# ActiveVisionLab/CrossScore

Measured on AMD Instinct MI355X. Metric: query-images/sec at 518x518, 5 ref views, bs=8; score-map MAE vs ref, higher is better.
Workload: dtype fp16

## Files before the change

### crossscore_amd/build.py

```python
from __future__ import annotations

import os
import subprocess
import sys

HERE = os.path.dirname(os.path.abspath(__file__))
CSRC = os.path.join(HERE, "csrc")
LIB = os.path.join(HERE, "libcrossscore_hip.so")
SOURCES = ["api.hip", "forward.hip", "ops.hip", "fit_host.hip", "gemm.hip", "gemm256.hip", "attention.hip", "refuse.hip", "elementwise.hip", "preprocess.hip", "panel.hip", "panel4.hip", "patch.hip", "rowln.hip", "png.hip", "pngdec.hip", "jpegdec.hip", "jpegprog.hip", "gtmap.hip", "gtsum.hip", "select.hip", "scorepool.hip", "sheet.hip", "headfit.hip", "tailfit.hip", "attnbwd.hip", "crossfit.hip", "layerfit.hip"]


EXTRA_FLAGS = {"panel.hip": ["-fno-slp-vectorize"], "panel4.hip": ["-fno-slp-vectorize"], "attention.hip": ["-fno-slp-vectorize"]}


def _hipcc() -> str:
    for c in (os.environ.get("HIPCC"), "/opt/rocm/bin/hipcc", "hipcc"):
        if c and (os.path.isabs(c) and os.path.exists(c) or not os.path.isabs(c)):
            return c
    return "hipcc"


def needs_build() -> bool:
    if not os.path.exists(LIB):
        return True
    t = os.path.getmtime(LIB)
    deps = [os.path.join(CSRC, f) for f in os.listdir(CSRC)] + [os.path.join(os.path.dirname(HERE), "include", "crossscore_hip.h")]
    return any(os.path.getmtime(d) > t for d in deps)


def compile_library(lib: str, extra=None, csrc: str = CSRC, objdir=None, verbose: bool = True) -> str:
    objdir = objdir or os.path.join(HERE, "build")
    os.makedirs(objdir, exist_ok=True)
    objs = []
    procs = []
    for s in SOURCES:
        o = os.path.join(objdir, s.replace(".hip", ".o"))
        objs.append(o)
        cmd = ([_hipcc(), "--offload-arch=gfx950", "-O3", "-std=c++17", "-fPIC", "-Wno-unused-value"] + EXTRA_FLAGS.get(s, []) + (extra or {}).get(s, []) +
               ["-c", os.path.join(csrc, s), "-o", o])
        procs.append((cmd, subprocess.Popen(cmd, stdout=subprocess.PIPE, stderr=subprocess.STDOUT, text=True)))
    for cmd, p in procs:
        out, _ = p.communicate()
        if p.returncode != 0:
            raise RuntimeError("hipcc failed: " + " ".join(cmd) + "\n" + out)
        if verbose and out.strip():
            print(out, file=sys.stderr)
    cmd = [_hipcc(), "--offload-arch=gfx950", "-shared", "-fPIC", "-o", lib] + objs
    r = subprocess.run(cmd, stdout=subprocess.PIPE, stderr=subprocess.STDOUT, text=True)
    if r.returncode != 0:
        raise RuntimeError("link failed: " + r.stdout)
    return lib


def build(force: bool = False, verbose: bool = True) -> str:
    if not force and not needs_build():
        return LIB
    return compile_library(LIB, verbose=verbose)


if __name__ == "__main__":
    print(build(force="--force" in sys.argv))
```

### crossscore_amd/csrc/rowln.hip

```cpp
#include "cs_common.h"
#include <atomic>

namespace {

__device__ __forceinline__ float rl_add_other_half(float x) {
  const auto r = __builtin_amdgcn_permlane32_swap(__float_as_uint(x), __float_as_uint(x), false, false);
  return __uint_as_float(r[0]) + __uint_as_float(r[1]);
}

template <int C, bool BF, int G2>
__global__ __launch_bounds__(C / 96 * 64) void cs_rowln_kernel(CsRowLnParams p) {
  constexpr int NW = C / 96, NT = NW * 64;
  constexpr bool NEXT = G2 > 0;
  constexpr int BK = 64, NSL = C / BK;
  constexpr int APITCH = C * 2 + 16;
  constexpr int WPITCH = BK * 2 + 16;
  constexpr int WBUF = C * WPITCH;
  constexpr int ACH = C / 8, WCH = BK / 8;
  constexpr int AIT = 64 * ACH / NT, WIT = C * WCH / NT;
  static_assert(64 * ACH % NT == 0 && C * WCH % NT == 0, "staging maps");
  extern __shared__ __attribute__((aligned(16))) char smem[];
  char* As = smem;
  char* Ws = smem + 64 * APITCH;
  float* red = reinterpret_cast<float*>(Ws + 2 * WBUF);
  const int tid = threadIdx.x;
  const int lane = tid & 63;
  const int wv = __builtin_amdgcn_readfirstlane(tid >> 6);
  const int j = lane & 31, h = lane >> 5;
  const int row0 = blockIdx.x * 64;
  const int col0 = wv * 96;
  uint4 wreg[WIT];
#define RL_LOAD_W(REG, WP, LDW, SL)                                                                                \
  _Pragma("unroll") for (int it = 0; it < WIT; ++it) {                                                         \
    const int c_ = tid + it * NT, r_ = c_ / WCH, ch_ = c_ - r_ * WCH;                                          \
    REG[it] = *reinterpret_cast<const uint4*>((WP) + (size_t)r_ * (LDW) + (SL) * BK + ch_ * 8);                \
  }
#define RL_WRITE_W(REG, BUF)                                                                                   \
  _Pragma("unroll") for (int it = 0; it < WIT; ++it) {                                                         \
    const int c_ = tid + it * NT, r_ = c_ / WCH, ch_ = c_ - r_ * WCH;                                          \
    *reinterpret_cast<uint4*>(Ws + (BUF) * WBUF + r_ * WPITCH + ch_ * 16) = REG[it];                           \
  }
  RL_LOAD_W(wreg, p.W, p.ldw, 0)
  {
    uint4 areg[AIT];
#pragma unroll
    for (int it = 0; it < AIT; ++it) {
      const int c = tid + it * NT, r = c / ACH, ch = c - r * ACH;
      areg[it] = *reinterpret_cast<const uint4*>(p.A + (size_t)min(row0 + r, p.M - 1) * p.lda + ch * 8);
    }
#pragma unroll
    for (int it = 0; it < AIT; ++it) {
      const int c = tid + it * NT, r = c / ACH, ch = c - r * ACH;
      *reinterpret_cast<uint4*>(As + r * APITCH + ch * 16) = areg[it];
    }
  }
#define RL_KSLICE(SLICE)                                                                                       \
  _Pragma("unroll") for (int ks = 0; ks < BK / 16; ++ks) {                                                     \
    h16x8_t a[2], w[3];                                                                                        \
    _Pragma("unroll") for (int rb = 0; rb < 2; ++rb)                                                           \
      a[rb] = *reinterpret_cast<const h16x8_t*>(a_rd + rb * 32 * APITCH + ((SLICE) * (BK / 16) + ks) * 32);    \
    _Pragma("unroll") for (int ct = 0; ct < 3; ++ct) w[ct] = *reinterpret_cast<const h16x8_t*>(w_rd + ct * 32 * WPITCH + ks * 32); \
    _Pragma("unroll") for (int rb = 0; rb < 2; ++rb)                                                           \
      _Pragma("unroll") for (int ct = 0; ct < 3; ++ct) acc[rb][ct] = mfma_32x32x16<BF>(w[ct], a[rb], acc[rb][ct]); \
  }
  RL_WRITE_W(wreg, 0)
  __syncthreads();
  f32x16_t acc[2][3];
#pragma unroll
  for (int rb = 0; rb < 2; ++rb)
#pragma unroll
    for (int ct = 0; ct < 3; ++ct)
#pragma unroll
      for (int e = 0; e < 16; ++e) acc[rb][ct][e] = 0.f;
  const char* a_rd = As + j * APITCH + h * 16;
  for (int sl = 0; sl < NSL; ++sl) {
    if (sl + 1 < NSL) { RL_LOAD_W(wreg, p.W, p.ldw, sl + 1) }
    const char* w_rd = Ws + (sl & 1) * WBUF + (col0 + j) * WPITCH + h * 16;
    RL_KSLICE(sl)
    if (sl + 1 < NSL) { RL_WRITE_W(wreg, (sl + 1) & 1) }
    __syncthreads();
  }
  f32x4_t gam[3][4], bet[3][4];
#pragma unroll
  for (int ct = 0; ct < 3; ++ct)
#pragma unroll
    for (int g = 0; g < 4; ++g) {
      const int c = col0 + 32 * ct + 8 * g + 4 * h;
      const f32x4_t b4 = *reinterpret_cast<const f32x4_t*>(p.bias + c);
      gam[ct][g] = *reinterpret_cast<const f32x4_t*>(p.gamma + c);
      bet[ct][g] = *reinterpret_cast<const f32x4_t*>(p.beta + c);
#pragma unroll
      for (int rb = 0; rb < 2; ++rb)
#pragma unroll
        for (int i = 0; i < 4; ++i) acc[rb][ct][4 * g + i] += b4[i];
    }
  if (p.resid) {
#pragma unroll
    for (int rb = 0; rb < 2; ++rb) {
      const float* rr = p.resid + (size_t)min(row0 + 32 * rb + j, p.M - 1) * p.ldr + col0 + 4 * h;
#pragma unroll
      for (int ct = 0; ct < 3; ++ct)
#pragma unroll
        for (int g = 0; g < 4; ++g) {
          const f32x4_t r4 = *reinterpret_cast<const f32x4_t*>(rr + 32 * ct + 8 * g);
#pragma unroll
          for (int i = 0; i < 4; ++i) acc[rb][ct][4 * g + i] += r4[i];
        }
    }
  }
  float mean[2], rstd[2];
#pragma unroll
  for (int rb = 0; rb < 2; ++rb) {
    float s = 0.f;
#pragma unroll
    for (int ct = 0; ct < 3; ++ct)
#pragma unroll
      for (int e = 0; e < 16; e += 4) s += (acc[rb][ct][e] + acc[rb][ct][e + 1]) + (acc[rb][ct][e + 2] + acc[rb][ct][e + 3]);
    s = rl_add_other_half(s);
    if (h == 0) red[(0 * NW + wv) * 64 + 32 * rb + j] = s;
  }
  __syncthreads();
#pragma unroll
  for (int rb = 0; rb < 2; ++rb) {
    float s = 0.f;
#pragma unroll
    for (int w2 = 0; w2 < NW; ++w2) s += red[(0 * NW + w2) * 64 + 32 * rb + j];
    mean[rb] = s * (1.0f / C);
    float q = 0.f;
#pragma unroll
    for (int ct = 0; ct < 3; ++ct)
#pragma unroll
      for (int e = 0; e < 16; ++e) {
        const float d = acc[rb][ct][e] - mean[rb];
        q = fmaf(d, d, q);
      }
    q = rl_add_other_half(q);
    if (h == 0) red[(1 * NW + wv) * 64 + 32 * rb + j] = q;
  }
  __syncthreads();
#pragma unroll
  for (int rb = 0; rb < 2; ++rb) {
    float q = 0.f;
#pragma unroll
    for (int w2 = 0; w2 < NW; ++w2) q += red[(1 * NW + w2) * 64 + 32 * rb + j];
    rstd[rb] = 1.0f / sqrtf(q * (1.0f / C) + p.eps);
  }
#pragma unroll
  for (int rb = 0; rb < 2; ++rb) {
    const int row = row0 + 32 * rb + j;
    if (row < p.M) {
      float* o32 = p.out_f32 ? p.out_f32 + (size_t)row * C + col0 + 4 * h : nullptr;
      h16_t* o16 = p.out_f16 ? p.out_f16 + (size_t)row * C + col0 + 4 * h : nullptr;
#pragma unroll
      for (int ct = 0; ct < 3; ++ct)
#pragma unroll
        for (int g = 0; g < 4; ++g) {
          f32x4_t y;
#pragma unroll
          for (int i = 0; i < 4; ++i) y[i] = (acc[rb][ct][4 * g + i] - mean[rb]) * rstd[rb] * gam[ct][g][i] + bet[ct][g][i];
          if (o32) *reinterpret_cast<f32x4_t*>(o32 + 32 * ct + 8 * g) = y;
          if (o16) {
            uint2 o;
            o.x = pack_o16x2<BF>(y[0], y[1]);
            o.y = pack_o16x2<BF>(y[2], y[3]);
            *reinterpret_cast<uint2*>(o16 + 32 * ct + 8 * g) = o;
          }
        }
    }
  }
  if constexpr (NEXT) {
#pragma unroll
    for (int rb = 0; rb < 2; ++rb) {
      char* arow = As + (32 * rb + j) * APITCH + (col0 + 4 * h) * 2;
#pragma unroll
      for (int ct = 0; ct < 3; ++ct)
#pragma unroll
        for (int g = 0; g < 4; ++g) {
          float y[4];
#pragma unroll
          for (int i = 0; i < 4; ++i) y[i] = (acc[rb][ct][4 * g + i] - mean[rb]) * rstd[rb] * gam[ct][g][i] + bet[ct][g][i];
          uint2 o;
          o.x = pack_o16x2<BF>(y[0], y[1]);
          o.y = pack_o16x2<BF>(y[2], y[3]);
          *reinterpret_cast<uint2*>(arow + (32 * ct + 8 * g) * 2) = o;
        }
    }
    RL_LOAD_W(wreg, p.W2, p.ldw2, 0)
    RL_WRITE_W(wreg, 0)
    __syncthreads();
    constexpr int nsl2 = G2 * NSL;
#pragma unroll
    for (int s2 = 0; s2 < nsl2; ++s2) {
      const int grp = s2 / NSL, sl = s2 - grp * NSL;
      if (sl == 0) {
#pragma unroll
        for (int rb = 0; rb < 2; ++rb)
#pragma unroll
          for (int ct = 0; ct < 3; ++ct)
#pragma unroll
            for (int e = 0; e < 16; ++e) acc[rb][ct][e] = 0.f;
      }
      if (s2 + 1 < nsl2) {
        const int g2 = (s2 + 1) / NSL, sn = (s2 + 1) - g2 * NSL;
        RL_LOAD_W(wreg, p.W2 + (size_t)g2 * C * p.ldw2, p.ldw2, sn)
      }
      const char* w_rd = Ws + (s2 & 1) * WBUF + (col0 + j) * WPITCH + h * 16;
      RL_KSLICE(sl)
      if (s2 + 1 < nsl2) { RL_WRITE_W(wreg, (s2 + 1) & 1) }
      __syncthreads();
      if (sl == NSL - 1) {
#pragma unroll
        for (int rb = 0; rb < 2; ++rb) {
          const int row = row0 + 32 * rb + j;
          if (row < p.M) {
            h16_t* o2 = p.out2 + (size_t)row * p.ld2 + grp * C + col0 + 4 * h;
            const float* b2 = p.bias2 + grp * C + col0 + 4 * h;
#pragma unroll
            for (int ct = 0; ct < 3; ++ct)
#pragma unroll
              for (int g = 0; g < 4; ++g) {
                const f32x4_t b4 = *reinterpret_cast<const f32x4_t*>(b2 + 32 * ct + 8 * g);
                float v[4];
#pragma unroll
                for (int i = 0; i < 4; ++i) {
                  v[i] = acc[rb][ct][4 * g + i] + b4[i];
                  if (p.act2 == 1) v[i] = fmaxf(v[i], 0.f);
                  if (p.act2 == 2) v[i] = v[i] >= 0.f ? v[i] : 0.01f * v[i];
                }
                uint2 o;
                o.x = pack_o16x2<BF>(v[0], v[1]);
                o.y = pack_o16x2<BF>(v[2], v[3]);
                *reinterpret_cast<uint2*>(o2 + 32 * ct + 8 * g) = o;
              }
          }
        }
      }
    }
  }
#undef RL_KSLICE
#undef RL_LOAD_W
#undef RL_WRITE_W
}

}

extern "C" int cs_rowln_supported(int C) { return C == 384; }

extern "C" const char* cs_rowln_check(const CsRowLnParams* p, int C) {
  if (!cs_rowln_supported(C)) return "linear + LayerNorm: built for C = 384";
  if (!p->A || !p->W || !p->bias || !p->gamma || !p->beta || (!p->out_f32 && !p->out_f16 && !p->n2)) return "linear + LayerNorm: null operand";
  if (p->n2) {
    if ((p->n2 != C && p->n2 != 3 * C) || p->act2 < 0 || p->act2 > 2) return "linear + LayerNorm: the second stage takes C or 3 C output columns and act2 in 0..2";
    if (!p->W2 || !p->bias2 || !p->out2) return "linear + LayerNorm: null operand (second stage)";
    if (p->ldw2 % 8 || p->ldw2 < C || p->ld2 % 4 || p->ld2 < p->n2) return "linear + LayerNorm: row strides must keep 16-byte rows (second stage)";
    if (((uintptr_t)p->W2 | (uintptr_t)p->bias2) & 15 || ((uintptr_t)p->out2 & 7)) return "linear + LayerNorm: operands must be 16-byte aligned (second stage)";
  }
  if (p->M <= 0) return "linear + LayerNorm: empty shape";
  if (p->lda % 8 || p->ldw % 8 || p->lda < C || p->ldw < C || (p->resid && (p->ldr % 4 || p->ldr < C))) return "linear + LayerNorm: row strides must keep 16-byte rows";
  if (((uintptr_t)p->A | (uintptr_t)p->W | (uintptr_t)p->bias | (uintptr_t)p->gamma | (uintptr_t)p->beta | (uintptr_t)p->resid | (uintptr_t)p->out_f32 |
       (uintptr_t)p->out_f16) & 15)
    return "linear + LayerNorm: operands must be 16-byte aligned";
  return nullptr;
}

extern "C" hipError_t cs_rowln_launch(const CsRowLnParams* p, int C, int bf16, hipStream_t st) {
  if (C != 384) return hipErrorInvalidValue;
  constexpr int CC = 384, NW = CC / 96;
  constexpr int lds = 64 * (CC * 2 + 16) + 2 * CC * (64 * 2 + 16) + 2 * NW * 64 * 4;
  static std::atomic<bool> attr_done[16];
  int dev = 0;
  if (hipGetDevice(&dev) != hipSuccess || dev < 0 || dev >= 16) return hipErrorInvalidDevice;
  if (!attr_done[dev]) {
    const void* fns[6] = {reinterpret_cast<const void*>(cs_rowln_kernel<384, true, 0>), reinterpret_cast<const void*>(cs_rowln_kernel<384, false, 0>),
                          reinterpret_cast<const void*>(cs_rowln_kernel<384, true, 1>), reinterpret_cast<const void*>(cs_rowln_kernel<384, false, 1>),
                          reinterpret_cast<const void*>(cs_rowln_kernel<384, true, 3>), reinterpret_cast<const void*>(cs_rowln_kernel<384, false, 3>)};
    for (const void* f : fns)
      if (hipError_t e = hipFuncSetAttribute(f, hipFuncAttributeMaxDynamicSharedMemorySize, lds); e != hipSuccess) return e;
    attr_done[dev] = true;
  }
  const dim3 grid((p->M + 63) / 64), block(NW * 64);
#define RL_GO(G) do { if (bf16) hipLaunchKernelGGL((cs_rowln_kernel<384, true, G>), grid, block, lds, st, *p);  \
                      else hipLaunchKernelGGL((cs_rowln_kernel<384, false, G>), grid, block, lds, st, *p); } while (0)
  if (p->n2 == 0) RL_GO(0);
  else if (p->n2 == CC) RL_GO(1);
  else if (p->n2 == 3 * CC) RL_GO(3);
  else return hipErrorInvalidValue;
#undef RL_GO
  return hipGetLastError();
}
```

Before: 1397.

## Rewrite fused linear+LayerNorm kernel with per-wave DMA weight ring and 16x16 MFMA tiles

Restructures the row-LayerNorm GEMM kernel from 4 waves over 64-row tiles with register-staged, double-buffered weight slices into 8 waves over 48-row tiles. Each wave streams its own weight columns through a 4-deep per-wave LDS ring using direct global-to-LDS loads, synchronised with explicit vmcnt/lgkm waits instead of block-wide syncthreads. Both stages, including the chained second GEMM, run as one fully unrolled compile-time pipeline, and MFMA switches from 32x32x16 to 16x16x32. The intent is to hide weight-load latency and cut barrier overhead and register pressure, at the cost of heavy inline asm, hand-counted wait values that are fragile, and more blocks with smaller row tiles.

```diff
diff --git a/crossscore_amd/build.py b/crossscore_amd/build.py
--- a/crossscore_amd/build.py
+++ b/crossscore_amd/build.py
@@ -10,7 +10,8 @@
 SOURCES = ["api.hip", "forward.hip", "ops.hip", "fit_host.hip", "gemm.hip", "gemm256.hip", "attention.hip", "refuse.hip", "elementwise.hip", "preprocess.hip", "panel.hip", "panel4.hip", "patch.hip", "rowln.hip", "png.hip", "pngdec.hip", "jpegdec.hip", "jpegprog.hip", "gtmap.hip", "gtsum.hip", "select.hip", "scorepool.hip", "sheet.hip", "headfit.hip", "tailfit.hip", "attnbwd.hip", "crossfit.hip", "layerfit.hip"]
 
 
-EXTRA_FLAGS = {"panel.hip": ["-fno-slp-vectorize"], "panel4.hip": ["-fno-slp-vectorize"], "attention.hip": ["-fno-slp-vectorize"]}
+EXTRA_FLAGS = {"panel.hip": ["-fno-slp-vectorize"], "panel4.hip": ["-fno-slp-vectorize"], "attention.hip": ["-fno-slp-vectorize"],
+               "rowln.hip": ["-fno-slp-vectorize"]}
 
 
 def _hipcc() -> str:
diff --git a/crossscore_amd/csrc/rowln.hip b/crossscore_amd/csrc/rowln.hip
--- a/crossscore_amd/csrc/rowln.hip
+++ b/crossscore_amd/csrc/rowln.hip
@@ -1,245 +1,252 @@
-#include "cs_common.h"
+#include "panel_shared.h"
 #include <atomic>
 
 namespace {
 
-__device__ __forceinline__ float rl_add_other_half(float x) {
-  const auto r = __builtin_amdgcn_permlane32_swap(__float_as_uint(x), __float_as_uint(x), false, false);
-  return __uint_as_float(r[0]) + __uint_as_float(r[1]);
+constexpr int RL_R = 48;
+constexpr int RL_NW = 8;
+constexpr int RL_BK = 32;
+constexpr int RL_NS = 4;
+constexpr int RL_D = RL_NS - 1;
+constexpr int RL_SLOT = 3 * PANEL_FRAG;
+
+template <int C> struct RlCfg {
+  static_assert(C == RL_NW * 48 && C % RL_BK == 0, "eight waves of 48 columns");
+  static constexpr int NSL = C / RL_BK;
+  static constexpr int A_BYTES = 3 * NSL * PANEL_FRAG;
+  static constexpr int RING_OFF = A_BYTES;
+  static constexpr int RED_OFF = RING_OFF + RL_NW * RL_NS * RL_SLOT;
+  static constexpr int LDS = RED_OFF + 2 * RL_NW * RL_R * 4;
+};
+
+typedef unsigned rl_u32x2_t __attribute__((ext_vector_type(2)));
+
+__device__ __forceinline__ float rl_add_groups(float x) {
+  const auto r = __builtin_amdgcn_permlane16_swap(__float_as_uint(x), __float_as_uint(x), false, false);
+  return add_other_half(__uint_as_float(r[0]) + __uint_as_float(r[1]));
+}
+__device__ __forceinline__ void rl_gload16(f32x4_t& r, const float* src) {
+  asm volatile("global_load_dwordx4 %0, %1, off" : "=v"(r) : "v"(src) : "memory");
+}
+__device__ __forceinline__ void rl_touch(f32x4_t& r) { asm volatile("" : "+v"(r)); }
+__device__ __forceinline__ void rl_lds_write4(unsigned addr, float v) { asm volatile("ds_write_b32 %0, %1" ::"v"(addr), "v"(v) : "memory"); }
+__device__ __forceinline__ void rl_lds_write8(unsigned addr, rl_u32x2_t v) { asm volatile("ds_write_b64 %0, %1" ::"v"(addr), "v"(v) : "memory"); }
+template <int OFF>
+__device__ __forceinline__ void rl_lds_read4(unsigned addr, float& v) {
+  asm volatile("ds_read_b32 %0, %1 offset:%2" : "=&v"(v) : "v"(addr), "n"(OFF) : "memory");
+}
+__device__ __forceinline__ float rl_sum_waves(unsigned addr) {
+  float x[RL_NW];
+  sfor<RL_NW>([&](auto w) { rl_lds_read4<decltype(w)::value * RL_R * 4>(addr, x[decltype(w)::value]); });
+  CS_LGKM(0);
+  return ((x[0] + x[1]) + (x[2] + x[3])) + ((x[4] + x[5]) + (x[6] + x[7]));
 }
 
 template <int C, bool BF, int G2>
-__global__ __launch_bounds__(C / 96 * 64) void cs_rowln_kernel(CsRowLnParams p) {
-  constexpr int NW = C / 96, NT = NW * 64;
+__global__ __launch_bounds__(RL_NW * 64) void cs_rowln_kernel(CsRowLnParams p) {
+  using Cfg = RlCfg<C>;
   constexpr bool NEXT = G2 > 0;
-  constexpr int BK = 64, NSL = C / BK;
-  constexpr int APITCH = C * 2 + 16;
-  constexpr int WPITCH = BK * 2 + 16;
-  constexpr int WBUF = C * WPITCH;
-  constexpr int ACH = C / 8, WCH = BK / 8;
-  constexpr int AIT = 64 * ACH / NT, WIT = C * WCH / NT;
-  static_assert(64 * ACH % NT == 0 && C * WCH % NT == 0, "staging maps");
+  constexpr int NSL = Cfg::NSL, T = NSL * (1 + G2);
   extern __shared__ __attribute__((aligned(16))) char smem[];
-  char* As = smem;
-  char* Ws = smem + 64 * APITCH;
-  float* red = reinterpret_cast<float*>(Ws + 2 * WBUF);
+  const unsigned lds0 = (unsigned)(size_t)CS_LDS_PTR(smem);
   const int tid = threadIdx.x;
   const int lane = tid & 63;
   const int wv = __builtin_amdgcn_readfirstlane(tid >> 6);
-  const int j = lane & 31, h = lane >> 5;
-  const int row0 = blockIdx.x * 64;
-  const int col0 = wv * 96;
-  uint4 wreg[WIT];
-#define RL_LOAD_W(REG, WP, LDW, SL)                                                                                \
-  _Pragma("unroll") for (int it = 0; it < WIT; ++it) {                                                         \
-    const int c_ = tid + it * NT, r_ = c_ / WCH, ch_ = c_ - r_ * WCH;                                          \
-    REG[it] = *reinterpret_cast<const uint4*>((WP) + (size_t)r_ * (LDW) + (SL) * BK + ch_ * 8);                \
-  }
-#define RL_WRITE_W(REG, BUF)                                                                                   \
-  _Pragma("unroll") for (int it = 0; it < WIT; ++it) {                                                         \
-    const int c_ = tid + it * NT, r_ = c_ / WCH, ch_ = c_ - r_ * WCH;                                          \
-    *reinterpret_cast<uint4*>(Ws + (BUF) * WBUF + r_ * WPITCH + ch_ * 16) = REG[it];                           \
-  }
-  RL_LOAD_W(wreg, p.W, p.ldw, 0)
-  {
-    uint4 areg[AIT];
-#pragma unroll
-    for (int it = 0; it < AIT; ++it) {
-      const int c = tid + it * NT, r = c / ACH, ch = c - r * ACH;
-      areg[it] = *reinterpret_cast<const uint4*>(p.A + (size_t)min(row0 + r, p.M - 1) * p.lda + ch * 8);
-    }
-#pragma unroll
-    for (int it = 0; it < AIT; ++it) {
-      const int c = tid + it * NT, r = c / ACH, ch = c - r * ACH;
-      *reinterpret_cast<uint4*>(As + r * APITCH + ch * 16) = areg[it];
-    }
-  }
-#define RL_KSLICE(SLICE)                                                                                       \
-  _Pragma("unroll") for (int ks = 0; ks < BK / 16; ++ks) {                                                     \
-    h16x8_t a[2], w[3];                                                                                        \
-    _Pragma("unroll") for (int rb = 0; rb < 2; ++rb)                                                           \
-      a[rb] = *reinterpret_cast<const h16x8_t*>(a_rd + rb * 32 * APITCH + ((SLICE) * (BK / 16) + ks) * 32);    \
-    _Pragma("unroll") for (int ct = 0; ct < 3; ++ct) w[ct] = *reinterpret_cast<const h16x8_t*>(w_rd + ct * 32 * WPITCH + ks * 32); \
-    _Pragma("unroll") for (int rb = 0; rb < 2; ++rb)                                                           \
-      _Pragma("unroll") for (int ct = 0; ct < 3; ++ct) acc[rb][ct] = mfma_32x32x16<BF>(w[ct], a[rb], acc[rb][ct]); \
-  }
-  RL_WRITE_W(wreg, 0)
-  __syncthreads();
-  f32x16_t acc[2][3];
-#pragma unroll
-  for (int rb = 0; rb < 2; ++rb)
-#pragma unroll
-    for (int ct = 0; ct < 3; ++ct)
-#pragma unroll
-      for (int e = 0; e < 16; ++e) acc[rb][ct][e] = 0.f;
-  const char* a_rd = As + j * APITCH + h * 16;
-  for (int sl = 0; sl < NSL; ++sl) {
-    if (sl + 1 < NSL) { RL_LOAD_W(wreg, p.W, p.ldw, sl + 1) }
-    const char* w_rd = Ws + (sl & 1) * WBUF + (col0 + j) * WPITCH + h * 16;
-    RL_KSLICE(sl)
-    if (sl + 1 < NSL) { RL_WRITE_W(wreg, (sl + 1) & 1) }
-    __syncthreads();
-  }
-  f32x4_t gam[3][4], bet[3][4];
-#pragma unroll
-  for (int ct = 0; ct < 3; ++ct)
-#pragma unroll
-    for (int g = 0; g < 4; ++g) {
-      const int c = col0 + 32 * ct + 8 * g + 4 * h;
-      const f32x4_t b4 = *reinterpret_cast<const f32x4_t*>(p.bias + c);
-      gam[ct][g] = *reinterpret_cast<const f32x4_t*>(p.gamma + c);
-      bet[ct][g] = *reinterpret_cast<const f32x4_t*>(p.beta + c);
-#pragma unroll
-      for (int rb = 0; rb < 2; ++rb)
-#pragma unroll
-        for (int i = 0; i < 4; ++i) acc[rb][ct][4 * g + i] += b4[i];
-    }
-  if (p.resid) {
-#pragma unroll
-    for (int rb = 0; rb < 2; ++rb) {
-      const float* rr = p.resid + (size_t)min(row0 + 32 * rb + j, p.M - 1) * p.ldr + col0 + 4 * h;
-#pragma unroll
-      for (int ct = 0; ct < 3; ++ct)
-#pragma unroll
-        for (int g = 0; g < 4; ++g) {
-          const f32x4_t r4 = *reinterpret_cast<const f32x4_t*>(rr + 32 * ct + 8 * g);
-#pragma unroll
-          for (int i = 0; i < 4; ++i) acc[rb][ct][4 * g + i] += r4[i];
+  const int j = lane & 15, g = lane >> 4;
+  const int row0 = blockIdx.x * RL_R;
+  const int col0 = wv * 48;
+  const unsigned a_rd = lds0 + lane * 16;
+  const unsigned ring = lds0 + Cfg::RING_OFF + wv * (RL_NS * RL_SLOT);
+  const unsigned w_rd = ring + lane * 16;
+  const unsigned red = lds0 + Cfg::RED_OFF + (wv * RL_R + j) * 4;
+  const unsigned red_rd = lds0 + Cfg::RED_OFF + j * 4;
+
+  f32x4_t b4[3], gam[3], bet[3], r4[3][3], b2[NEXT ? G2 : 1][3];
+  int rowc[3];
+#pragma unroll
+  for (int rt = 0; rt < 3; ++rt) rowc[rt] = min(row0 + 16 * rt + j, p.M - 1);
+#pragma unroll
+  for (int ct = 0; ct < 3; ++ct) {
+    const int c = col0 + 16 * ct + 4 * g;
+    rl_gload16(b4[ct], p.bias + c);
+    rl_gload16(gam[ct], p.gamma + c);
+    rl_gload16(bet[ct], p.beta + c);
+  }
+#pragma unroll
+  for (int rt = 0; rt < 3; ++rt)
+#pragma unroll
+    for (int ct = 0; ct < 3; ++ct) {
+      const int c = col0 + 16 * ct + 4 * g;
+      rl_gload16(r4[rt][ct], p.resid ? p.resid + (size_t)rowc[rt] * p.ldr + c : p.bias + c);
+    }
+  if constexpr (NEXT) {
+#pragma unroll
+    for (int grp = 0; grp < G2; ++grp)
+#pragma unroll
+      for (int ct = 0; ct < 3; ++ct) rl_gload16(b2[grp][ct], p.bias2 + grp * C + col0 + 16 * ct + 4 * g);
+  }
+#pragma unroll
+  for (int rt = 0; rt < 3; ++rt) {
+    const char* src = reinterpret_cast<const char*>(p.A + (size_t)rowc[rt] * p.lda + 8 * g);
+    dma_piece<0>(src + wv * 64, lds0 + (rt * NSL + wv) * PANEL_FRAG);
+    if (wv < NSL - RL_NW) dma_piece<0>(src + (wv + RL_NW) * 64, lds0 + (rt * NSL + wv + RL_NW) * PANEL_FRAG);
+  }
+  const char* wsrc[3];
+  const char* w2src[3];
+#pragma unroll
+  for (int ct = 0; ct < 3; ++ct) {
+    wsrc[ct] = reinterpret_cast<const char*>(p.W + (size_t)(col0 + 16 * ct + j) * p.ldw + 8 * g);
+    w2src[ct] = NEXT ? reinterpret_cast<const char*>(p.W2 + (size_t)(col0 + 16 * ct + j) * p.ldw2 + 8 * g) : nullptr;
+  }
+  auto issue = [&](auto tc) {
+    constexpr int t = decltype(tc)::value;
+    if constexpr (t < T) {
+      constexpr int slot = t % RL_NS, grp = t < NSL ? 0 : (t - NSL) / NSL, s = t % NSL;
+      sfor<3>([&](auto ct_) {
+        constexpr int ct = decltype(ct_)::value;
+        const char* src = t < NSL ? wsrc[ct] + s * 64 : w2src[ct] + ((size_t)grp * C * p.ldw2 + s * RL_BK) * 2;
+        dma_piece<0>(src, ring + slot * RL_SLOT + ct * PANEL_FRAG);
+      });
+    }
+  };
+  h16x8_t wf[2][3], af[2][3];
+  auto read_frags = [&](auto tc) {
+    constexpr int t = decltype(tc)::value;
+    constexpr int slot = t % RL_NS, s = t % NSL, b = t & 1;
+    sfor<3>([&](auto i_) {
+      constexpr int i = decltype(i_)::value;
+      lds_read1<slot * RL_SLOT + i * PANEL_FRAG>(w_rd, wf[b][i]);
+      lds_read1<(i * NSL + s) * PANEL_FRAG>(a_rd, af[b][i]);
+    });
+  };
+  sfor<RL_D>([&](auto tc) { issue(tc); });
+  CS_VMCNT(3 * RL_D);
+  __builtin_amdgcn_s_barrier();
+#pragma unroll
+  for (int ct = 0; ct < 3; ++ct) {
+    rl_touch(b4[ct]); rl_touch(gam[ct]); rl_touch(bet[ct]);
+#pragma unroll
+    for (int rt = 0; rt < 3; ++rt) rl_touch(r4[rt][ct]);
+    if constexpr (NEXT) {
+#pragma unroll
+      for (int grp = 0; grp < G2; ++grp) rl_touch(b2[grp][ct]);
+    }
+  }
+  CS_VMCNT(3 * (RL_D - 1));
+  read_frags(IC<0>{});
+  CS_LGKM(0);
+
+  f32x4_t acc[3][3];
+  float mean[3], rstd[3];
+  sfor<T>([&](auto tc) {
+    constexpr int t = decltype(tc)::value;
+    constexpr int s = t % NSL;
+    constexpr bool ahead = t + 1 < T && t + 1 != NSL;
+    if constexpr (s == 0) {
+#pragma unroll
+      for (int rt = 0; rt < 3; ++rt)
+#pragma unroll
+        for (int ct = 0; ct < 3; ++ct) acc[rt][ct] = f32x4_t{0.f, 0.f, 0.f, 0.f};
+    }
+    issue(IC<t + RL_D>{});
+    if constexpr (ahead) {
+      constexpr int last = t + RL_D < T - 1 ? t + RL_D : T - 1;
+      CS_VMCNT(3 * (last - (t + 1)));
+      read_frags(IC<t + 1>{});
+      CS_SB();
+    }
+#pragma unroll
+    for (int rt = 0; rt < 3; ++rt)
+#pragma unroll
+      for (int ct = 0; ct < 3; ++ct) acc[rt][ct] = mfma_16x16x32<BF>(wf[t & 1][ct], af[t & 1][rt], acc[rt][ct]);
+    CS_SB();
+    CS_LGKM(0);
+
+    if constexpr (t == NSL - 1) {
+#pragma unroll
+      for (int rt = 0; rt < 3; ++rt)
+#pragma unroll
+        for (int ct = 0; ct < 3; ++ct) {
+          acc[rt][ct] += b4[ct];
+          if (p.resid) acc[rt][ct] += r4[rt][ct];
         }
-    }
-  }
-  float mean[2], rstd[2];
-#pragma unroll
-  for (int rb = 0; rb < 2; ++rb) {
-    float s = 0.f;
-#pragma unroll
-    for (int ct = 0; ct < 3; ++ct)
-#pragma unroll
-      for (int e = 0; e < 16; e += 4) s += (acc[rb][ct][e] + acc[rb][ct][e + 1]) + (acc[rb][ct][e + 2] + acc[rb][ct][e + 3]);
-    s = rl_add_other_half(s);
-    if (h == 0) red[(0 * NW + wv) * 64 + 32 * rb + j] = s;
-  }
-  __syncthreads();
-#pragma unroll
-  for (int rb = 0; rb < 2; ++rb) {
-    float s = 0.f;
-#pragma unroll
-    for (int w2 = 0; w2 < NW; ++w2) s += red[(0 * NW + w2) * 64 + 32 * rb + j];
-    mean[rb] = s * (1.0f / C);
-    float q = 0.f;
-#pragma unroll
-    for (int ct = 0; ct < 3; ++ct)
-#pragma unroll
-      for (int e = 0; e < 16; ++e) {
-        const float d = acc[rb][ct][e] - mean[rb];
-        q = fmaf(d, d, q);
-      }
-    q = rl_add_other_half(q);
-    if (h == 0) red[(1 * NW + wv) * 64 + 32 * rb + j] = q;
-  }
-  __syncthreads();
-#pragma unroll
-  for (int rb = 0; rb < 2; ++rb) {
-    float q = 0.f;
-#pragma unroll
-    for (int w2 = 0; w2 < NW; ++w2) q += red[(1 * NW + w2) * 64 + 32 * rb + j];
-    rstd[rb] = 1.0f / sqrtf(q * (1.0f / C) + p.eps);
-  }
-#pragma unroll
-  for (int rb = 0; rb < 2; ++rb) {
-    const int row = row0 + 32 * rb + j;
-    if (row < p.M) {
-      float* o32 = p.out_f32 ? p.out_f32 + (size_t)row * C + col0 + 4 * h : nullptr;
-      h16_t* o16 = p.out_f16 ? p.out_f16 + (size_t)row * C + col0 + 4 * h : nullptr;
-#pragma unroll
-      for (int ct = 0; ct < 3; ++ct)
-#pragma unroll
-        for (int g = 0; g < 4; ++g) {
+#pragma unroll
+      for (int rt = 0; rt < 3; ++rt) {
+        float part[3];
+#pragma unroll
+        for (int ct = 0; ct < 3; ++ct) part[ct] = (acc[rt][ct][0] + acc[rt][ct][1]) + (acc[rt][ct][2] + acc[rt][ct][3]);
+        const float sum = rl_add_groups((part[0] + part[1]) + part[2]);
+        if (g == 0) rl_lds_write4(red + 16 * rt * 4, sum);
+      }
+      CS_LGKM(0);
+      __builtin_amdgcn_s_barrier();
+#pragma unroll
+      for (int rt = 0; rt < 3; ++rt) {
+        mean[rt] = rl_sum_waves(red_rd + 16 * rt * 4) * (1.0f / C);
+        float q = 0.f;
+#pragma unroll
+        for (int ct = 0; ct < 3; ++ct)
+#pragma unroll
+          for (int i = 0; i < 4; ++i) {
+            const float d = acc[rt][ct][i] - mean[rt];
+            q = fmaf(d, d, q);
+          }
+        q = rl_add_groups(q);
+        if (g == 0) rl_lds_write4(red + (RL_NW * RL_R + 16 * rt) * 4, q);
+      }
+      CS_LGKM(0);
+      __builtin_amdgcn_s_barrier();
+#pragma unroll
+      for (int rt = 0; rt < 3; ++rt) rstd[rt] = 1.0f / sqrtf(rl_sum_waves(red_rd + (RL_NW * RL_R + 16 * rt) * 4) * (1.0f / C) + p.eps);
+#pragma unroll
+      for (int rt = 0; rt < 3; ++rt) {
+        const int row = row0 + 16 * rt + j;
+        float* o32 = p.out_f32 && row < p.M ? p.out_f32 + (size_t)row * C + col0 + 4 * g : nullptr;
+        h16_t* o16 = p.out_f16 && row < p.M ? p.out_f16 + (size_t)row * C + col0 + 4 * g : nullptr;
+#pragma unroll
+        for (int ct = 0; ct < 3; ++ct) {
           f32x4_t y;
 #pragma unroll
-          for (int i = 0; i < 4; ++i) y[i] = (acc[rb][ct][4 * g + i] - mean[rb]) * rstd[rb] * gam[ct][g][i] + bet[ct][g][i];
-          if (o32) *reinterpret_cast<f32x4_t*>(o32 + 32 * ct + 8 * g) = y;
-          if (o16) {
-            uint2 o;
-            o.x = pack_o16x2<BF>(y[0], y[1]);
-            o.y = pack_o16x2<BF>(y[2], y[3]);
-            *reinterpret_cast<uint2*>(o16 + 32 * ct + 8 * g) = o;
+          for (int i = 0; i < 4; ++i) y[i] = (acc[rt][ct][i] - mean[rt]) * rstd[rt] * gam[ct][i] + bet[ct][i];
+          const rl_u32x2_t o = {pack_o16x2<BF>(y[0], y[1]), pack_o16x2<BF>(y[2], y[3])};
+          if (o32) *reinterpret_cast<f32x4_t*>(o32 + 16 * ct) = y;
+          if (o16) *reinterpret_cast<rl_u32x2_t*>(o16 + 16 * ct) = o;
+          if constexpr (NEXT) {
+            const int f = col0 + 16 * ct + 4 * g;
+            rl_lds_write8(lds0 + (rt * NSL + (f >> 5)) * PANEL_FRAG + (j + 16 * ((f & 31) >> 3)) * 16 + (f & 7) * 2, o);
           }
         }
-    }
-  }
-  if constexpr (NEXT) {
-#pragma unroll
-    for (int rb = 0; rb < 2; ++rb) {
-      char* arow = As + (32 * rb + j) * APITCH + (col0 + 4 * h) * 2;
-#pragma unroll
-      for (int ct = 0; ct < 3; ++ct)
-#pragma unroll
-        for (int g = 0; g < 4; ++g) {
-          float y[4];
-#pragma unroll
-          for (int i = 0; i < 4; ++i) y[i] = (acc[rb][ct][4 * g + i] - mean[rb]) * rstd[rb] * gam[ct][g][i] + bet[ct][g][i];
-          uint2 o;
-          o.x = pack_o16x2<BF>(y[0], y[1]);
-          o.y = pack_o16x2<BF>(y[2], y[3]);
-          *reinterpret_cast<uint2*>(arow + (32 * ct + 8 * g) * 2) = o;
-        }
-    }
-    RL_LOAD_W(wreg, p.W2, p.ldw2, 0)
-    RL_WRITE_W(wreg, 0)
-    __syncthreads();
-    constexpr int nsl2 = G2 * NSL;
-#pragma unroll
-    for (int s2 = 0; s2 < nsl2; ++s2) {
-      const int grp = s2 / NSL, sl = s2 - grp * NSL;
-      if (sl == 0) {
-#pragma unroll
-        for (int rb = 0; rb < 2; ++rb)
-#pragma unroll
-          for (int ct = 0; ct < 3; ++ct)
-#pragma unroll
-            for (int e = 0; e < 16; ++e) acc[rb][ct][e] = 0.f;
-      }
-      if (s2 + 1 < nsl2) {
-        const int g2 = (s2 + 1) / NSL, sn = (s2 + 1) - g2 * NSL;
-        RL_LOAD_W(wreg, p.W2 + (size_t)g2 * C * p.ldw2, p.ldw2, sn)
-      }
-      const char* w_rd = Ws + (s2 & 1) * WBUF + (col0 + j) * WPITCH + h * 16;
-      RL_KSLICE(sl)
-      if (s2 + 1 < nsl2) { RL_WRITE_W(wreg, (s2 + 1) & 1) }
-      __syncthreads();
-      if (sl == NSL - 1) {
-#pragma unroll
-        for (int rb = 0; rb < 2; ++rb) {
-          const int row = row0 + 32 * rb + j;
-          if (row < p.M) {
-            h16_t* o2 = p.out2 + (size_t)row * p.ld2 + grp * C + col0 + 4 * h;
-            const float* b2 = p.bias2 + grp * C + col0 + 4 * h;
-#pragma unroll
-            for (int ct = 0; ct < 3; ++ct)
-#pragma unroll
-              for (int g = 0; g < 4; ++g) {
-                const f32x4_t b4 = *reinterpret_cast<const f32x4_t*>(b2 + 32 * ct + 8 * g);
-                float v[4];
-#pragma unroll
-                for (int i = 0; i < 4; ++i) {
-                  v[i] = acc[rb][ct][4 * g + i] + b4[i];
-                  if (p.act2 == 1) v[i] = fmaxf(v[i], 0.f);
-                  if (p.act2 == 2) v[i] = v[i] >= 0.f ? v[i] : 0.01f * v[i];
-                }
-                uint2 o;
-                o.x = pack_o16x2<BF>(v[0], v[1]);
-                o.y = pack_o16x2<BF>(v[2], v[3]);
-                *reinterpret_cast<uint2*>(o2 + 32 * ct + 8 * g) = o;
-              }
+      }
+      if constexpr (NEXT) {
+        CS_LGKM(0);
+        __builtin_amdgcn_s_barrier();
+        CS_VMCNT(3 * ((NSL - 1 + RL_D < T - 1 ? NSL - 1 + RL_D : T - 1) - NSL));
+        read_frags(IC<NSL>{});
+        CS_LGKM(0);
+      }
+    }
+    if constexpr (NEXT && t >= NSL && s == NSL - 1) {
+      constexpr int grp = (t - NSL) / NSL;
+#pragma unroll
+      for (int rt = 0; rt < 3; ++rt) {
+        const int row = row0 + 16 * rt + j;
+        if (row < p.M) {
+          h16_t* o2 = p.out2 + (size_t)row * p.ld2 + grp * C + col0 + 4 * g;
+#pragma unroll
+          for (int ct = 0; ct < 3; ++ct) {
+            float v[4];
+#pragma unroll
+            for (int i = 0; i < 4; ++i) {
+              v[i] = acc[rt][ct][i] + b2[grp][ct][i];
+              if (p.act2 == 1) v[i] = fmaxf(v[i], 0.f);
+              if (p.act2 == 2) v[i] = v[i] >= 0.f ? v[i] : 0.01f * v[i];
+            }
+            *reinterpret_cast<rl_u32x2_t*>(o2 + 16 * ct) = rl_u32x2_t{pack_o16x2<BF>(v[0], v[1]), pack_o16x2<BF>(v[2], v[3])};
           }
         }
       }
     }
-  }
-#undef RL_KSLICE
-#undef RL_LOAD_W
-#undef RL_WRITE_W
+  });
 }
 
 }
@@ -265,8 +272,7 @@
 
 extern "C" hipError_t cs_rowln_launch(const CsRowLnParams* p, int C, int bf16, hipStream_t st) {
   if (C != 384) return hipErrorInvalidValue;
-  constexpr int CC = 384, NW = CC / 96;
-  constexpr int lds = 64 * (CC * 2 + 16) + 2 * CC * (64 * 2 + 16) + 2 * NW * 64 * 4;
+  constexpr int lds = RlCfg<384>::LDS;
   static std::atomic<bool> attr_done[16];
   int dev = 0;
   if (hipGetDevice(&dev) != hipSuccess || dev < 0 || dev >= 16) return hipErrorInvalidDevice;
@@ -278,12 +284,12 @@
       if (hipError_t e = hipFuncSetAttribute(f, hipFuncAttributeMaxDynamicSharedMemorySize, lds); e != hipSuccess) return e;
     attr_done[dev] = true;
   }
-  const dim3 grid((p->M + 63) / 64), block(NW * 64);
+  const dim3 grid((p->M + RL_R - 1) / RL_R), block(RL_NW * 64);
 #define RL_GO(G) do { if (bf16) hipLaunchKernelGGL((cs_rowln_kernel<384, true, G>), grid, block, lds, st, *p);  \
                       else hipLaunchKernelGGL((cs_rowln_kernel<384, false, G>), grid, block, lds, st, *p); } while (0)
   if (p->n2 == 0) RL_GO(0);
-  else if (p->n2 == CC) RL_GO(1);
-  else if (p->n2 == 3 * CC) RL_GO(3);
+  else if (p->n2 == 3 * 384) RL_GO(3);
+  else if (p->n2 == 384) RL_GO(1);
   else return hipErrorInvalidValue;
 #undef RL_GO
   return hipGetLastError();
```

Measured after the change: 1394. No clear change (-0.2%).
